# suous/RecNeXt

Hardware: AMD Instinct MI355X
Metric: images/sec RecNeXt-M3 224x224 bf16 (higher is better)
Workload: dtype bf16

## Files before the change

### recnext_amd/csrc/rcx_api.hip

```cpp
#include "../../include/recnext_amd.h"
#include "rcx_opts.h"
#include "rcx_launch.h"

#include <cstdarg>
#include <initializer_list>
#include <cstdio>
#include <cstdlib>

namespace {

thread_local char g_err[512] = "";

int fail(int code, const char* fmt, ...)
{
    va_list ap;
    va_start(ap, fmt);
    vsnprintf(g_err, sizeof(g_err), fmt, ap);
    va_end(ap);
    return code;
}

int hip_fail(hipError_t e, const char* what, const char* prefix = "")
{
    snprintf(g_err, sizeof(g_err), "%s%s: %s", prefix, what, hipGetErrorString(e));
// ... 935 lines not shown
    return e == hipSuccess ? 0 : hip_fail(e, "rcx_recattn_qkcore_fwd");
}

int rcx_recattn_down_qkcore_supported(int B, int H, int W, int C, int heads, int x_dtype)
{
    if (B <= 0 || H <= 0 || W <= 0 || C <= 0 || heads <= 0 || C % heads) return 0;
    return rcx::recattn_down_qkcore_applicable(B, H, W, C, heads, x_dtype) ? 1 : 0;
}

int rcx_recattn_down_qkcore_fwd(const void* x, const float* w_down_kkc, const float* b_down, const void* wqk_bf16, const float* bqk,
                                const float* w_pe_kkc, const float* b_pe, float* out, int B, int H, int W, int C, int heads, int x_dtype, void* stream)
{
    if (!x || !w_down_kkc || !wqk_bf16 || !bqk || !w_pe_kkc || !out) return fail(RCX_ERR_BAD_ARG, "rcx_recattn_down_qkcore_fwd: null pointer");
    if (B <= 0 || H <= 0 || W <= 0 || C <= 0 || heads <= 0) return fail(RCX_ERR_BAD_ARG, "non-positive extent B=%d H=%d W=%d C=%d heads=%d", B, H, W, C, heads);
    if (C % heads) return fail(RCX_ERR_BAD_ARG, "C=%d is not a multiple of heads=%d", C, heads);
    if (!known_dtype(x_dtype)) return fail(RCX_ERR_BAD_ARG, "unknown dtype %d", x_dtype);
    if (((size_t)wqk_bf16 & 15) || ((size_t)out & 15) || ((size_t)bqk & 15) || ((size_t)w_pe_kkc & 15) || ((size_t)b_pe & 15))
        return fail(RCX_ERR_BAD_ARG, "rcx_recattn_down_qkcore_fwd: wqk, bqk, w_pe_kkc, b_pe and out must be 16-byte aligned");
    if (!rcx::recattn_down_qkcore_applicable(B, H, W, C, heads, x_dtype))
        return fail(RCX_ERR_UNSUPPORTED, "rcx_recattn_down_qkcore_fwd: %d x %d plane, %d heads of %d, dtype %d: the one-launch form takes the 14 x 14 plane (1 .. 8 heads) "
                                         "and the 7 x 7 plane (1 .. 16 heads) of bf16 / f16 activations, heads of 4 .. 32 channels, or 2, 4 or 8 heads of 36 .. 64 in fours "
                                         "whose image fits the LDS (use rcx_dwconv2d_fwd + rcx_recattn_qkcore_fwd)",
                    H, W, heads, C / heads, x_dtype);
    hipError_t e = rcx::recattn_down_qkcore(x, w_down_kkc, b_down, wqk_bf16, bqk, w_pe_kkc, b_pe, out, B, H, C, heads, x_dtype, (hipStream_t)stream);
    return e == hipSuccess ? 0 : hip_fail(e, "rcx_recattn_down_qkcore_fwd");
}

int rcx_recattn2d_fwd_supported(int B, int H, int W, int C, int heads, int mode, int dtype)
{
    if (B <= 0 || H <= 0 || W <= 0 || C <= 0 || heads <= 0 || C % heads) return 0;
    return rcx::recattn2d_unit_applicable(B, H, W, C, heads, dtype, mode == RCX_MODE_NEAREST ? 1 : 0) ? 1 : 0;
}

int rcx_recattn2d_fwd(const void* x, void* y, const float* w_down_kkc, const float* b_down, const void* wqk_bf16, const float* bqk,
                      const float* w_pe_kkc, const float* b_pe, const float* w_conv_kkc, const float* b_conv,
                      int B, int H, int W, int C, int heads, int mode, int dtype, void* stream)
{
    if (!x || !y || !w_down_kkc || !wqk_bf16 || !bqk || !w_pe_kkc || !w_conv_kkc) return fail(RCX_ERR_BAD_ARG, "rcx_recattn2d_fwd: null pointer");
    if (B <= 0 || H <= 0 || W <= 0 || C <= 0 || heads <= 0) return fail(RCX_ERR_BAD_ARG, "non-positive extent B=%d H=%d W=%d C=%d heads=%d", B, H, W, C, heads);
    if (C % heads) return fail(RCX_ERR_BAD_ARG, "C=%d is not a multiple of heads=%d", C, heads);
    if (!known_dtype(dtype)) return fail(RCX_ERR_BAD_ARG, "unknown dtype %d", dtype);
    if (mode != RCX_MODE_BILINEAR && mode != RCX_MODE_NEAREST) return fail(RCX_ERR_BAD_ARG, "unknown mode %d", mode);
    if (((size_t)wqk_bf16 & 15) || ((size_t)bqk & 15) || ((size_t)w_pe_kkc & 15) || ((size_t)b_pe & 15))
        return fail(RCX_ERR_BAD_ARG, "rcx_recattn2d_fwd: wqk, bqk, w_pe_kkc and b_pe must be 16-byte aligned");
    if (!rcx::recattn2d_unit_applicable(B, H, W, C, heads, dtype, mode == RCX_MODE_NEAREST ? 1 : 0))
        return fail(RCX_ERR_UNSUPPORTED, "rcx_recattn2d_fwd: %d x %d plane, %d heads of %d, mode %d, dtype %d: the one-launch unit takes the 14 x 14 (1 .. 8 heads) and 7 x 7 (1 .. 16 heads) planes of bf16 / f16 "
                                         "activations, heads of 32 or 4 .. 28 channels (not above 32), nearest resize (use rcx_recattn_down_qkcore_fwd / rcx_dwconv2d_fwd + rcx_recattn_qkcore_fwd, then "
                                         "rcx_upadd_dwconv_fwd)", H, W, heads, C / heads, mode, dtype);
    hipError_t e = rcx::recattn2d_unit(x, w_down_kkc, b_down, wqk_bf16, bqk, w_pe_kkc, b_pe, w_conv_kkc, b_conv, y, B, H, C, heads, dtype, (hipStream_t)stream);
    return e == hipSuccess ? 0 : hip_fail(e, "rcx_recattn2d_fwd");
}

int rcx_stem_supported(int N, int H, int W, int CM, int CO, int dtype) { return rcx::stem_applicable(N, H, W, CM, CO, dtype) ? 1 : 0; }

size_t rcx_stem_pack_bytes(int CM, int CO) { return rcx::stem_pack_bytes(CM, CO); }

int rcx_stem_fwd(const void* x, void* y, const void* w1frag, const float* b1, const void* w2frag, const float* b2, int N, int H, int W, int CM, int CO, int dtype, void* stream)
{
    if (!x || !y || !w1frag || !b1 || !w2frag || !b2) return fail(RCX_ERR_BAD_ARG, "rcx_stem_fwd: null pointer");
    if (N <= 0 || H <= 0 || W <= 0 || CM <= 0 || CO <= 0) return fail(RCX_ERR_BAD_ARG, "non-positive extent N=%d H=%d W=%d CM=%d CO=%d", N, H, W, CM, CO);
    if (!known_dtype(dtype)) return fail(RCX_ERR_BAD_ARG, "unknown dtype %d", dtype);
    if (((size_t)x & 1) || ((size_t)y & 7) || ((size_t)w1frag & 15) || ((size_t)b1 & 15) || ((size_t)w2frag & 15) || ((size_t)b2 & 15))
        return fail(RCX_ERR_BAD_ARG, "rcx_stem_fwd: w1frag, b1, w2frag and b2 must be 16-byte aligned, y 8-byte aligned");
    if (!rcx::stem_applicable(N, H, W, CM, CO, dtype))
        return fail(RCX_ERR_UNSUPPORTED, "rcx_stem_fwd: no kernel for CM=%d CO=%d dtype %d (bf16; CM in {20, 24, 28, 32, 40}, CO %% 4 == 0, CO <= 96; one image of x below 2^31 bytes)", CM, CO, dtype);
    hipError_t e = rcx::stem_fwd(x, y, w1frag, b1, w2frag, b2, N, H, W, CM, CO, dtype, (hipStream_t)stream);
    return e == hipSuccess ? 0 : hip_fail(e, "rcx_stem_fwd");
}

int rcx_channel_mlp_supported(int M, int C, int H, int dtype) { return rcx::channel_mlp_applicable(M, C, H, dtype) ? 1 : 0; }

size_t rcx_channel_mlp_pack_bytes(int C, int H) { return rcx::channel_mlp_pack_bytes(C, H); }

int rcx_channel_mlp_fwd(const void* z, const void* x, void* y, const void* wfrag, const float* bias, int M, int C, int H, int dtype, void* stream)
{
    if (!z || !x || !y || !wfrag || !bias) return fail(RCX_ERR_BAD_ARG, "rcx_channel_mlp_fwd: null pointer");
    if (M <= 0 || C <= 0 || H <= 0) return fail(RCX_ERR_BAD_ARG, "non-positive extent M=%d C=%d H=%d", M, C, H);
    if (!known_dtype(dtype)) return fail(RCX_ERR_BAD_ARG, "unknown dtype %d", dtype);
    if (((size_t)z & 15) || ((size_t)x & 7) || ((size_t)y & 7) || ((size_t)wfrag & 15) || ((size_t)bias & 15))
        return fail(RCX_ERR_BAD_ARG, "rcx_channel_mlp_fwd: z, wfrag and bias must be 16-byte aligned, x and y 8-byte aligned");
    if (y == z || y == x) return fail(RCX_ERR_BAD_ARG, "rcx_channel_mlp_fwd: y must not alias its inputs");
    if (!rcx::channel_mlp_applicable(M, C, H, dtype))
        return fail(RCX_ERR_UNSUPPORTED, "rcx_channel_mlp_fwd: no kernel for M=%d C=%d H=%d dtype %d (bf16; (C, H) = (40 | 48, 96), (56 | 64, 128), (80, 160), (96, 192), (128, 256), (160, 320), "
                                         "(192, 384), (256, 512), (320, 640); M C 2 < 2^31)", M, C, H, dtype);
    hipError_t e = rcx::channel_mlp(z, x, y, wfrag, bias, M, C, H, dtype, (hipStream_t)stream);
    return e == hipSuccess ? 0 : hip_fail(e, "rcx_channel_mlp_fwd");
}

int rcx_ls_recattn_supported(int B, int H, int W, int C, int split, int heads, int dtype)
{
    return rcx::ls_recattn_applicable(B, H, W, C, split, heads, dtype) ? 1 : 0;
}

int rcx_ls_la3_supported(int B, int H, int W, int C, int split, int heads, int dtype)
{
    return rcx::ls_la3_applicable(B, H, W, C, split, heads, dtype) ? 1 : 0;
}

namespace {
bool any_misaligned(std::initializer_list<const void*> ps)
{
    for (const void* p : ps)
        if ((size_t)p & 15) return true;
    return false;
}
}

int rcx_ls_recattn_fwd(const void* x, void* r, void* t, const float* w_rep, const float* b_rep, const float* w_down_kkc, const float* b_down,
                       const float* wqT, const float* bq, const float* wkT, const float* bk, const float* w_pe_kkc, const float* b_pe,
                       const float* w_conv_kkc, const float* b_conv, int B, int H, int W, int C, int split, int heads, int dtype, void* stream)
{
    if (!x || !r || !t || !w_rep || !b_rep || !w_down_kkc || !b_down || !wqT || !bq || !wkT || !bk || !w_pe_kkc || !b_pe || !w_conv_kkc || !b_conv)
        return fail(RCX_ERR_BAD_ARG, "rcx_ls_recattn_fwd: null pointer");
    if (B <= 0 || H <= 0 || W <= 0 || C <= 0 || split <= 0 || heads <= 0)
        return fail(RCX_ERR_BAD_ARG, "non-positive extent B=%d H=%d W=%d C=%d split=%d heads=%d", B, H, W, C, split, heads);
    if (!known_dtype(dtype)) return fail(RCX_ERR_BAD_ARG, "unknown dtype %d", dtype);
    if (r == x || t == x || r == t) return fail(RCX_ERR_BAD_ARG, "rcx_ls_recattn_fwd: r and t must alias neither x nor each other");
    if (any_misaligned({x, r, t, w_rep, b_rep, w_down_kkc, b_down, wqT, bq, wkT, bk, w_pe_kkc, b_pe, w_conv_kkc, b_conv}))
        return fail(RCX_ERR_BAD_ARG, "rcx_ls_recattn_fwd: every tensor must be 16-byte aligned");
    if (!rcx::ls_recattn_applicable(B, H, W, C, split, heads, dtype))
        return fail(RCX_ERR_UNSUPPORTED, "rcx_ls_recattn_fwd: %d x %d plane, C=%d, split=%d, %d heads: one head, C and split multiples of 4, and an image whose slice "
                                         "mixer fits the LDS", H, W, C, split, heads);
    hipError_t e = rcx::ls_recattn_fwd(x, r, t, w_rep, b_rep, w_down_kkc, b_down, wqT, bq, wkT, bk, w_pe_kkc, b_pe, w_conv_kkc, b_conv,
                                       B, H, W, C, split, dtype, (hipStream_t)stream);
    return e == hipSuccess ? 0 : hip_fail(e, "rcx_ls_recattn_fwd");
}

int rcx_ls_la3_fwd(const void* x, void* r, void* t, const float* w_rep, const float* b_rep, const float* wqT, const float* bq,
                   const float* wkT, const float* bk, const float* w_pe_kkc, const float* b_pe, int B, int H, int W, int C, int split, int heads,
                   int dtype, void* stream)
{
    if (!x || !r || !t || !w_rep || !b_rep || !wqT || !bq || !wkT || !bk || !w_pe_kkc || !b_pe) return fail(RCX_ERR_BAD_ARG, "rcx_ls_la3_fwd: null pointer");
    if (B <= 0 || H <= 0 || W <= 0 || C <= 0 || split <= 0 || heads <= 0)
        return fail(RCX_ERR_BAD_ARG, "non-positive extent B=%d H=%d W=%d C=%d split=%d heads=%d", B, H, W, C, split, heads);
    if (!known_dtype(dtype)) return fail(RCX_ERR_BAD_ARG, "unknown dtype %d", dtype);
    if (r == x || t == x || r == t) return fail(RCX_ERR_BAD_ARG, "rcx_ls_la3_fwd: r and t must alias neither x nor each other");
    if (any_misaligned({x, r, t, w_rep, b_rep, wqT, bq, wkT, bk, w_pe_kkc, b_pe}))
        return fail(RCX_ERR_BAD_ARG, "rcx_ls_la3_fwd: every tensor must be 16-byte aligned");
    if (!rcx::ls_la3_applicable(B, H, W, C, split, heads, dtype))
        return fail(RCX_ERR_UNSUPPORTED, "rcx_ls_la3_fwd: %d x %d plane, C=%d, split=%d, %d heads: at most 64 tokens, C and split multiples of 4, split a multiple "
                                         "of 2 heads", H, W, C, split, heads);
    hipError_t e = rcx::ls_la3_fwd(x, r, t, w_rep, b_rep, wqT, bq, wkT, bk, w_pe_kkc, b_pe, B, H, W, C, split, heads, dtype, (hipStream_t)stream);
    return e == hipSuccess ? 0 : hip_fail(e, "rcx_ls_la3_fwd");
}

int rcx_ls_recattn_tiled_supported(int B, int H, int W, int C, int split, int heads, int dtype)
{
    return rcx::ls_recattn_tiled_applicable(B, H, W, C, split, heads, dtype) ? 1 : 0;
}

int rcx_ls_la3_tiled_supported(int B, int H, int W, int C, int split, int heads, int dtype)
{
    return rcx::ls_la3_tiled_applicable(B, H, W, C, split, heads, dtype) ? 1 : 0;
}

size_t rcx_ls_recattn_tiled_workspace_bytes(int B, int H, int W, int C, int split, int heads, int dtype)
{
    return rcx::ls_recattn_tiled_workspace_bytes(B, H, W, C, split, heads, dtype);
}

size_t rcx_ls_la3_tiled_workspace_bytes(int B, int H, int W, int C, int split, int heads, int dtype)
{
    return rcx::ls_la3_tiled_workspace_bytes(B, H, W, C, split, heads, dtype);
}

namespace {
int check_ls_tiled(const char* fn, std::initializer_list<const void*> ps, const void* x, const void* r, const void* t, const void* workspace,
// ... 98 lines not shown
```

### recnext_amd/csrc/rcx_mlp.hip

```cpp
#include "rcx_common.h"
#include "rcx_launch.h"
#include "rcx_gelu.h"

namespace rcx {
namespace mlp {

typedef float f32x16 __attribute__((ext_vector_type(16)));
typedef float f32x4q __attribute__((ext_vector_type(4)));
typedef float f32x2q __attribute__((ext_vector_type(2)));
typedef __bf16 bf16x8 __attribute__((ext_vector_type(8)));
typedef __bf16 bf16x4 __attribute__((ext_vector_type(4)));
typedef unsigned u32x4q __attribute__((ext_vector_type(4)));
typedef unsigned u32x2q __attribute__((ext_vector_type(2)));

__device__ __forceinline__ void wave_sync()
{
    __builtin_amdgcn_fence(__ATOMIC_RELEASE, "wavefront");
    __builtin_amdgcn_wave_barrier();
    __builtin_amdgcn_fence(__ATOMIC_ACQUIRE, "wavefront");
}

template <int KS1, int CT, int RD>
__device__ __forceinline__ void hidden_tile_ring(const u32x4q* Lc, const float* b1t, int lane, int h, const bf16x8 (&zb)[KS1], f32x16 (&d2)[CT])
{
    constexpr int R1 = KS1 < RD ? KS1 : RD, N2 = 2 * CT, R2 = N2 < RD ? N2 : RD;
    u32x4q ring[RD];
#pragma unroll
    for (int j = 0; j < R1; ++j) ring[j] = Lc[j * 64 + lane];
    f32x16 d1;
#pragma unroll
    for (int i = 0; i < 16; ++i) d1[i] = 0.f;
#pragma unroll
    for (int ks = 0; ks < KS1; ++ks) {
        const bf16x8 a = __builtin_bit_cast(bf16x8, ring[ks % R1]);
        if (ks + R1 < KS1) ring[ks % R1] = Lc[(ks + R1) * 64 + lane];
        d1 = __builtin_amdgcn_mfma_f32_32x32x16_bf16(a, zb[ks], d1, 0, 0, 0);
    }
#pragma unroll
    for (int f = 0; f < R2; ++f) ring[f] = Lc[(KS1 + 2 * (f % CT) + f / CT) * 64 + lane];
    bf16x8 hb[2];
    gelu_f32x2 gv[8];
#pragma unroll
    for (int g = 0; g < 4; ++g) {
        const f32x4q bb = *reinterpret_cast<const f32x4q*>(b1t + 8 * g + 4 * h);
        gv[2 * g] = gelu_f32x2{d1[4 * g] + bb.x, d1[4 * g + 1] + bb.y};
        gv[2 * g + 1] = gelu_f32x2{d1[4 * g + 2] + bb.z, d1[4 * g + 3] + bb.w};
    }
    {
        gelu_f32x2 ga[4] = {gv[0], gv[1], gv[2], gv[3]}, gb[4] = {gv[4], gv[5], gv[6], gv[7]};
        gelu2x_batch<4>(ga);
        gelu2x_batch<4>(gb);
#pragma unroll
        for (int i = 0; i < 4; ++i) { gv[i] = ga[i]; gv[4 + i] = gb[i]; }
    }
#pragma unroll
    for (int g = 0; g < 4; ++g) {
        hb[g >> 1][4 * (g & 1) + 0] = (__bf16)gv[2 * g].x; hb[g >> 1][4 * (g & 1) + 1] = (__bf16)gv[2 * g].y;
        hb[g >> 1][4 * (g & 1) + 2] = (__bf16)gv[2 * g + 1].x; hb[g >> 1][4 * (g & 1) + 3] = (__bf16)gv[2 * g + 1].y;
    }
#pragma unroll
    for (int f = 0; f < N2; ++f) {
        const bf16x8 a = __builtin_bit_cast(bf16x8, ring[f % R2]);
        if (f + R2 < N2) ring[f % R2] = Lc[(KS1 + 2 * ((f + R2) % CT) + (f + R2) / CT) * 64 + lane];
        d2[f % CT] = __builtin_amdgcn_mfma_f32_32x32x16_bf16(a, hb[f / CT], d2[f % CT], 0, 0, 0);
    }
}


template <int KS1, int HT, int CT, int NW, int WPS, bool KX, bool OX, bool STAGED>
__global__ void __launch_bounds__(64 * NW, WPS)
k_channel_mlp(const bf16_t* __restrict__ z, const bf16_t* __restrict__ xres, bf16_t* __restrict__ y, const u32x4q* __restrict__ wfrag, const float* __restrict__ bias,
              int M, int C, int ntiles)
{
    extern __shared__ __attribute__((aligned(16))) unsigned char lds_raw[];
    constexpr int NF = HT * KS1 + CT * 2 * HT;
    const u32x4q* const Lf = reinterpret_cast<const u32x4q*>(lds_raw);
    const float* const Lb1 = reinterpret_cast<const float*>(lds_raw + (size_t)NF * 1024);
    const float* const Lb2 = Lb1 + 32 * HT;
    {
        u32x4q* Lw = reinterpret_cast<u32x4q*>(lds_raw);
        for (int i = threadIdx.x; i < NF * 64; i += 64 * NW) Lw[i] = wfrag[i];
        float* Lb = reinterpret_cast<float*>(lds_raw + (size_t)NF * 1024);
        for (int i = threadIdx.x; i < 32 * (HT + CT); i += 64 * NW) Lb[i] = bias[i];
    }
    __syncthreads();
// ... 269 lines not shown
        const u32x4q* src = wfrag + (size_t)chunk * NCH * 64 + threadIdx.x;
        u32x4q* dst = Lring + (size_t)slot * NCH * 64 + wv * 64;
#pragma unroll
        for (int i = 0; i < PER; ++i)
            __builtin_amdgcn_global_load_lds((__attribute__((address_space(1))) void*)(src + i * NT), (__attribute__((address_space(3))) void*)(dst + i * NT), 16, 0, 0);
    };
    constexpr int VM_ALL = 0x70, VM_NEXT = 0x70 | (PER & 15) | ((PER >> 4) << 14);
    fill(0, 0);
    fill(1, 1);
    for (int i = threadIdx.x; i < 32 * (HT + CT); i += NT) Lb1[i] = bias[i];
    const unsigned nbytes = (unsigned)M * (unsigned)C * 2u;
    const __amdgpu_buffer_rsrc_t zsrc = __builtin_amdgcn_make_buffer_rsrc((void*)z, 0, nbytes, 0x00020000);
    const __amdgpu_buffer_rsrc_t xsrc = __builtin_amdgcn_make_buffer_rsrc((void*)xres, 0, nbytes, 0x00020000);
    const __amdgpu_buffer_rsrc_t ysrc = __builtin_amdgcn_make_buffer_rsrc((void*)y, 0, nbytes, 0x00020000);
    const unsigned zo0 = (unsigned)(lane >> 3) * RB + 16u * (lane & 7), za0 = (unsigned)(lane >> 3) * ZP + 16u * (lane & 7);
    const unsigned ot = lane >> 2, ob = 16u * (lane & 3);
    if (!(__builtin_popcount(wv) & 1)) __builtin_amdgcn_s_setprio(1);
    int slot = 0;
    for (int block = blockIdx.x; block < nblocks; block += gridDim.x) {
        const unsigned base = (unsigned)(32 * (block * NW + wave)) * (unsigned)RB;
        const bool more = block + (int)gridDim.x < nblocks;
        bf16x8 zb[KS1];
        {
            u32x4q zq[KS1];
#pragma unroll
            for (int i = 0; i < KS1; ++i)
                zq[i] = __builtin_bit_cast(u32x4q, __builtin_amdgcn_raw_buffer_load_b128(zsrc, (int)(base + zo0 + 8u * RB * (i % KH) + RBH * (i / KH)), 0, 0));
#pragma unroll
            for (int q = 0; q < ZH; ++q) {
#pragma unroll
                for (int i = 0; i < KH; ++i) *reinterpret_cast<u32x4q*>(Lt + za0 + 8 * ZP * i) = zq[q * KH + i];
                wave_sync();
#pragma unroll
                for (int k = 0; k < KH; ++k) zb[q * KH + k] = __builtin_bit_cast(bf16x8, *reinterpret_cast<const u32x4q*>(Lt + r * ZP + 32 * k + 16 * h));
                wave_sync();
            }
        }
        f32x16 d2[CT];
#pragma unroll
        for (int ct = 0; ct < CT; ++ct)
#pragma unroll
            for (int i = 0; i < 16; ++i) d2[ct][i] = 0.f;
#pragma unroll 1
        for (int ht = 0; ht < HT; ++ht) {
            if (ht + 1 < HT || more) __builtin_amdgcn_s_waitcnt(VM_NEXT);
            else __builtin_amdgcn_s_waitcnt(VM_ALL);
            __builtin_amdgcn_s_barrier();
            if (ht + 2 < HT || more) fill((ht + 2) % HT, slot == 0 ? 2 : slot - 1);
            hidden_tile_ring<KS1, CT, 4>(Lring + (size_t)slot * NCH * 64, Lb1 + 32 * ht, lane, h, zb, d2);
            slot = slot == NS - 1 ? 0 : slot + 1;
        }
        u32x4q xq[CT][2];
#pragma unroll
        for (int ct = 0; ct < CT; ++ct)
#pragma unroll
            for (int j = 0; j < 2; ++j)
                xq[ct][j] = __builtin_bit_cast(u32x4q, __builtin_amdgcn_raw_buffer_load_b128(xsrc, (int)(base + (16u * j + ot) * RB + 64u * ct + ob), 0, 0));
#pragma unroll
        for (int ct = 0; ct < CT; ++ct) {
#pragma unroll
            for (int g = 0; g < 4; ++g) {
                const f32x4q bb = *reinterpret_cast<const f32x4q*>(Lb2 + 32 * ct + 8 * g + 4 * h);
                *reinterpret_cast<f32x4q*>(Lt + r * OP + 4 * (8 * g + 4 * h)) =
                    f32x4q{d2[ct][4 * g] + bb.x, d2[ct][4 * g + 1] + bb.y, d2[ct][4 * g + 2] + bb.z, d2[ct][4 * g + 3] + bb.w};
            }
            wave_sync();
#pragma unroll
            for (int j = 0; j < 2; ++j) {
                const unsigned char* src = Lt + (16 * j + ot) * OP + 2 * ob;
                const f32x4q lo = *reinterpret_cast<const f32x4q*>(src), hi = *reinterpret_cast<const f32x4q*>(src + 16);
                const u32x4q xv = xq[ct][j];
                bf16x8 o;
                o[0] = (__bf16)(lo.x + __uint_as_float(xv.x << 16)); o[1] = (__bf16)(lo.y + __uint_as_float(xv.x & 0xffff0000u));
                o[2] = (__bf16)(lo.z + __uint_as_float(xv.y << 16)); o[3] = (__bf16)(lo.w + __uint_as_float(xv.y & 0xffff0000u));
                o[4] = (__bf16)(hi.x + __uint_as_float(xv.z << 16)); o[5] = (__bf16)(hi.y + __uint_as_float(xv.z & 0xffff0000u));
                o[6] = (__bf16)(hi.z + __uint_as_float(xv.w << 16)); o[7] = (__bf16)(hi.w + __uint_as_float(xv.w & 0xffff0000u));
                __builtin_amdgcn_raw_buffer_store_b128(__builtin_bit_cast(u32x4q, o), ysrc, (int)(base + (16u * j + ot) * RB + 64u * ct + ob), 0, 0);
            }
            wave_sync();
        }
    }
}

}

static bool mlp_shape(int C, int H, int* ks1, int* ht, int* ct)
{
    if (C <= 0 || H <= 0 || C % 8 || H % 32) return false;
    *ks1 = (C + 15) / 16; *ht = H / 32; *ct = (C + 31) / 32;
    if (C > 128 && (*ct & 1)) ++*ct;
    return true;
}

bool channel_mlp_applicable(int M, int C, int H, int dtype)
{
    int ks1, ht, ct;
    if (dtype != 1 || M <= 0 || !mlp_shape(C, H, &ks1, &ht, &ct)) return false;
    if ((unsigned long long)M * C * 2 >= (1ull << 31)) return false;
    if (C == 256 && ht == 16) return true;
    if (C == 192 && ht == 12) return true;
    if ((C == 160 && ht == 10) || (C == 320 && ht == 20)) return true;
    return (ks1 == 4 && ht == 4 && ct == 2) || (C == 128 && ht == 8) || (ks1 == 3 && ht == 3 && ct == 2) || (C == 96 && ht == 6) || (C == 80 && ht == 5);
}

size_t channel_mlp_pack_bytes(int C, int H)
{
    int ks1, ht, ct;
    if (!mlp_shape(C, H, &ks1, &ht, &ct)) return 0;
    return (size_t)(ht * ks1 + ct * 2 * ht) * 1024;
}

template <int KS1, int HT, int CT, bool KX, bool OX>
static hipError_t launch_mlp(const void* z, const void* x, void* y, const void* wfrag, const float* bias, int M, int C, int ncu, hipStream_t s)
{
    constexpr size_t lds = (size_t)(HT * KS1 + CT * 2 * HT) * 1024 + sizeof(float) * 32 * (HT + CT);
    static_assert(lds <= 160 * 1024, "the weights must fit the LDS");
    constexpr int NW = CT <= 2 ? 12 : 8, WPS = NW / 4;
    constexpr bool STAGED = CT <= 2;
    constexpr size_t stage = STAGED ? (size_t)NW * 32 * ((32 * KS1 + 16) > (128 * CT + 16) ? (32 * KS1 + 16) : (128 * CT + 16)) : 0;
    if ((C == 16 * KS1) != KX || (C == 32 * CT) != OX) return hipErrorInvalidConfiguration;
    auto kfn = mlp::k_channel_mlp<KS1, HT, CT, NW, WPS, KX, OX, STAGED>;
    static_assert(lds + stage <= 160 * 1024, "weights + the waves' images must fit the LDS");
    RCX_SET_LDS_ONCE(kfn, lds + stage);
    const int ntiles = (M + 31) / 32;
    int grid = ncu;
    if (grid * NW > ntiles) grid = (ntiles + NW - 1) / NW;
    hipLaunchKernelGGL(kfn, dim3((unsigned)grid), dim3(64 * NW), lds + stage, s, (const bf16_t*)z, (const bf16_t*)x, (bf16_t*)y, (const mlp::u32x4q*)wfrag, bias, M, C, ntiles);
    return hipGetLastError();
}

template <int KS1, int HT, int CT, int NW, int ZH = 1, bool ZPF = true>
static hipError_t launch_mlp_stream(const void* z, const void* x, void* y, const void* wfrag, const float* bias, int M, int C, int ncu, hipStream_t s)
{
    constexpr int NCH = KS1 + 2 * CT, ZP = 32 * KS1 / ZH + 16, OP = 256 + 16, IMG = 32 * (ZP > OP ? ZP : OP);
    constexpr size_t lds = (size_t)2 * NCH * 1024 + sizeof(float) * 32 * (HT + CT) + (size_t)NW * IMG;
    static_assert(lds <= 160 * 1024, "the ring and the waves' images must fit the LDS");
    static_assert(CT % 2 == 0 && 32 * CT >= 16 * KS1 && 32 * (CT - 2) < 16 * KS1, "output tiles: the channel count rounded up to a multiple of 64");
    if (C != 16 * KS1) return hipErrorInvalidConfiguration;
    auto kfn = mlp::k_channel_mlp_stream<KS1, HT, CT, NW, NW / 4, ZH, ZPF>;
    RCX_SET_LDS_ONCE(kfn, lds);
    const int nblocks = (M + 32 * NW - 1) / (32 * NW);
    const int grid = nblocks < ncu ? nblocks : ncu;
    hipLaunchKernelGGL(kfn, dim3((unsigned)grid), dim3(64 * NW), lds, s, (const bf16_t*)z, (const bf16_t*)x, (bf16_t*)y, (const mlp::u32x4q*)wfrag, bias, M, C, nblocks);
    return hipGetLastError();
}

static hipError_t launch_mlp_pair256(const void* z, const void* x, void* y, const void* wfrag, const float* bias, int M, int C, int ncu, hipStream_t s)
{
    constexpr int KS1 = 16, HT = 16, CT = 8, NCH = KS1 + 2 * CT, IMG = 32 * (128 + 16);
    constexpr size_t lds = (size_t)3 * NCH * 1024 + sizeof(float) * 32 * (HT + CT) + (size_t)8 * IMG;
    static_assert(lds <= 160 * 1024, "the ring and the waves' images must fit the LDS");
    if (C != 16 * KS1) return hipErrorInvalidConfiguration;
    auto kfn = mlp::k_channel_mlp_pair<KS1, HT, CT>;
    RCX_SET_LDS_ONCE(kfn, lds);
    const int nblocks = (M + 255) / 256;
    const int grid = nblocks < ncu ? nblocks : ncu;
    hipLaunchKernelGGL(kfn, dim3((unsigned)grid), dim3(512), lds, s, (const bf16_t*)z, (const bf16_t*)x, (bf16_t*)y, (const mlp::u32x4q*)wfrag, bias, M, C, nblocks);
    return hipGetLastError();
}

hipError_t channel_mlp(const void* z, const void* x, void* y, const void* wfrag, const float* bias, int M, int C, int H, int dtype, hipStream_t s)
{
    int ks1, ht, ct;
    if (!channel_mlp_applicable(M, C, H, dtype) || !mlp_shape(C, H, &ks1, &ht, &ct)) return hipErrorInvalidConfiguration;
    static std::atomic<int> cus[RCX_MAX_DEVICES];
    int dev = 0, ncu = 256;
    if (hipGetDevice(&dev) == hipSuccess && dev >= 0 && dev < RCX_MAX_DEVICES) {
        ncu = cus[dev].load(std::memory_order_relaxed);
        if (ncu <= 0) {
            int v = 0;
            ncu = hipDeviceGetAttribute(&v, hipDeviceAttributeMultiprocessorCount, dev) == hipSuccess && v > 0 ? v : 256;
            cus[dev].store(ncu, std::memory_order_relaxed);
        }
    }
    if (C == 256 && ht == 16) return launch_mlp_pair256(z, x, y, wfrag, bias, M, C, ncu, s);
    if (C == 192 && ht == 12) return launch_mlp_stream<12, 12, 6, 4>(z, x, y, wfrag, bias, M, C, ncu, s);
    if (C == 160 && ht == 10) return launch_mlp_stream<10, 10, 6, 4>(z, x, y, wfrag, bias, M, C, ncu, s);
    if (C == 320 && ht == 20) return launch_mlp_stream<20, 20, 10, 4, 2, false>(z, x, y, wfrag, bias, M, C, ncu, s);
    if (ks1 == 4 && ht == 4) return C == 64 ? launch_mlp<4, 4, 2, true, true>(z, x, y, wfrag, bias, M, C, ncu, s)
                                            : launch_mlp<4, 4, 2, false, false>(z, x, y, wfrag, bias, M, C, ncu, s);
    if (ks1 == 8 && ht == 8) {
        if (C != 128) return hipErrorInvalidConfiguration;
        return launch_mlp_stream<8, 8, 4, 8>(z, x, y, wfrag, bias, M, C, ncu, s);
    }
    if (ks1 == 3 && ht == 3) return C == 48 ? launch_mlp<3, 3, 2, true, false>(z, x, y, wfrag, bias, M, C, ncu, s)
                                            : launch_mlp<3, 3, 2, false, false>(z, x, y, wfrag, bias, M, C, ncu, s);
    if (ks1 == 6 && ht == 6) return C == 96 ? launch_mlp<6, 6, 3, true, true>(z, x, y, wfrag, bias, M, C, ncu, s) : hipErrorInvalidConfiguration;
    if (ks1 == 5 && ht == 5) return C == 80 ? launch_mlp<5, 5, 3, true, false>(z, x, y, wfrag, bias, M, C, ncu, s) : hipErrorInvalidConfiguration;
    return hipErrorInvalidConfiguration;
}

}
```

Baseline: 109,800.

## Add fused channel-MLP kernel for C=512 with streamed weight fragments

After: 113,200 (median of 6 runs). 3.1% higher.

```diff
diff --git a/recnext_amd/csrc/rcx_api.hip b/recnext_amd/csrc/rcx_api.hip
--- a/recnext_amd/csrc/rcx_api.hip
+++ b/recnext_amd/csrc/rcx_api.hip
@@ -1041,7 +1041,7 @@
     if (y == z || y == x) return fail(RCX_ERR_BAD_ARG, "rcx_channel_mlp_fwd: y must not alias its inputs");
     if (!rcx::channel_mlp_applicable(M, C, H, dtype))
         return fail(RCX_ERR_UNSUPPORTED, "rcx_channel_mlp_fwd: no kernel for M=%d C=%d H=%d dtype %d (bf16; (C, H) = (40 | 48, 96), (56 | 64, 128), (80, 160), (96, 192), (128, 256), (160, 320), "
-                                         "(192, 384), (256, 512), (320, 640); M C 2 < 2^31)", M, C, H, dtype);
+                                         "(192, 384), (256, 512), (320, 640), (512, 1024) from a minimum M upward; M C 2 < 2^31)", M, C, H, dtype);
     hipError_t e = rcx::channel_mlp(z, x, y, wfrag, bias, M, C, H, dtype, (hipStream_t)stream);
     return e == hipSuccess ? 0 : hip_fail(e, "rcx_channel_mlp_fwd");
 }
diff --git a/recnext_amd/csrc/rcx_mlp.hip b/recnext_amd/csrc/rcx_mlp.hip
--- a/recnext_amd/csrc/rcx_mlp.hip
+++ b/recnext_amd/csrc/rcx_mlp.hip
@@ -1,6 +1,7 @@
 #include "rcx_common.h"
 #include "rcx_launch.h"
 #include "rcx_gelu.h"
+#include <type_traits>
 
 namespace rcx {
 namespace mlp {
@@ -436,6 +437,178 @@
     }
 }
 
+
+template <int KS1, int HT, int CT, int RD>
+__global__ void __launch_bounds__(512, 2)
+k_channel_mlp_wide(const bf16_t* __restrict__ z, const bf16_t* __restrict__ xres, bf16_t* __restrict__ y, const u32x4q* __restrict__ wfrag, const float* __restrict__ bias, int M)
+{
+    extern __shared__ __attribute__((aligned(16))) unsigned char lds_raw[];
+    constexpr int NW = 8, NT = 64 * NW, SH = 8, NST = HT / SH, NCH = KS1 + 2 * CT, NF = KS1 + 4 * SH;
+    static_assert(CT == 2 * NW && HT % SH == 0 && SH == NW && NF % RD == 0 && KS1 % RD == 0 && KS1 % 8 == 0, "a hidden tile (phase A) and two output tiles (phase B) per wave");
+    constexpr int RB = 32 * KS1, OP = 256 + 16, IMG = 32 * OP;
+    constexpr int ZBYTES = 2 * KS1 * 1024, XBYTES = SH * 4 * 1024;
+    static_assert(NW * IMG <= ZBYTES + XBYTES, "the output images alias the z fragments and exchange buffer 0");
+    u32x4q* const Lz = reinterpret_cast<u32x4q*>(lds_raw);
+    u32x4q* const Lx = reinterpret_cast<u32x4q*>(lds_raw + ZBYTES);
+    float* const Lb1 = reinterpret_cast<float*>(lds_raw + ZBYTES + 2 * XBYTES);
+    const float* const Lb2 = Lb1 + 32 * HT;
+    const int lane = threadIdx.x & 63, r = lane & 31, h = lane >> 5;
+    const int wv = __builtin_amdgcn_readfirstlane(threadIdx.x >> 6);
+    auto frag = [&](int s, int i) -> u32x4q {
+        const int ht = SH * s + (i < KS1 ? wv : (i - KS1) >> 2);
+        const int f = i < KS1 ? i : KS1 + 4 * wv + 2 * ((i - KS1) & 1) + (((i - KS1) >> 1) & 1);
+        return wfrag[((size_t)ht * NCH + f) * 64 + lane];
+    };
+    u32x4q ring[RD];
+#pragma unroll
+    for (int i = 0; i < RD; ++i) ring[i] = frag(0, i);
+    const unsigned nbytes = (unsigned)M * (unsigned)RB;
+    const __amdgpu_buffer_rsrc_t zsrc = __builtin_amdgcn_make_buffer_rsrc((void*)z, 0, nbytes, 0x00020000);
+    const __amdgpu_buffer_rsrc_t xsrc = __builtin_amdgcn_make_buffer_rsrc((void*)xres, 0, nbytes, 0x00020000);
+    const __amdgpu_buffer_rsrc_t ysrc = __builtin_amdgcn_make_buffer_rsrc((void*)y, 0, nbytes, 0x00020000);
+    const unsigned base = blockIdx.x * 64u * RB;
+    {
+        const unsigned go = base + (8u * wv + (lane & 7)) * RB + 16u * (lane >> 3);
+        u32x4q zq[KS1 / 4];
+#pragma unroll
+        for (int j = 0; j < KS1 / 4; ++j) zq[j] = __builtin_bit_cast(u32x4q, __builtin_amdgcn_raw_buffer_load_b128(zsrc, (int)(go + 128u * j), 0, 0));
+        for (int i = threadIdx.x; i < 32 * (HT + CT); i += NT) Lb1[i] = bias[i];
+        u32x4q* const dst = Lz + ((wv >> 2) * KS1 + (lane >> 4)) * 64 + ((lane >> 3) & 1) * 32 + 8 * (wv & 3) + (lane & 7);
+#pragma unroll
+        for (int j = 0; j < KS1 / 4; ++j) dst[4 * j * 64] = zq[j];
+    }
+    __syncthreads();
+    if (!(__builtin_popcount(wv) & 1)) __builtin_amdgcn_s_setprio(1);
+    constexpr int LGKM0 = 0xC07F;
+    f32x16 d2[2][2];
+#pragma unroll
+    for (int c2 = 0; c2 < 2; ++c2)
+#pragma unroll
+        for (int tt = 0; tt < 2; ++tt)
+#pragma unroll
+            for (int i = 0; i < 16; ++i) d2[c2][tt][i] = 0.f;
+    const unsigned ot = lane >> 3, ob = 16u * (lane & 7);
+    u32x4q xq[2][4];
+    auto step = [&](int s, auto last_c) {
+        constexpr bool LAST = decltype(last_c)::value;
+        const int sn = LAST ? 0 : s + 1;
+        f32x16 d1[2];
+#pragma unroll
+        for (int tt = 0; tt < 2; ++tt)
+#pragma unroll
+            for (int i = 0; i < 16; ++i) d1[tt][i] = 0.f;
+        constexpr int BD = 2;
+        u32x4q zb[BD][2];
+#pragma unroll
+        for (int k = 0; k < BD; ++k)
+#pragma unroll
+            for (int tt = 0; tt < 2; ++tt) zb[k][tt] = Lz[(tt * KS1 + k) * 64 + lane];
+#pragma unroll
+        for (int ks = 0; ks < KS1; ++ks) {
+            const bf16x8 a = __builtin_bit_cast(bf16x8, ring[ks % RD]);
+            ring[ks % RD] = frag(s, ks + RD);
+            const bf16x8 b0 = __builtin_bit_cast(bf16x8, zb[ks % BD][0]), b1 = __builtin_bit_cast(bf16x8, zb[ks % BD][1]);
+            if (ks + BD < KS1) {
+#pragma unroll
+                for (int tt = 0; tt < 2; ++tt) zb[ks % BD][tt] = Lz[(tt * KS1 + ks + BD) * 64 + lane];
+            }
+            d1[0] = __builtin_amdgcn_mfma_f32_32x32x16_bf16(a, b0, d1[0], 0, 0, 0);
+            d1[1] = __builtin_amdgcn_mfma_f32_32x32x16_bf16(a, b1, d1[1], 0, 0, 0);
+            __builtin_amdgcn_sched_barrier(0);
+        }
+        const float* const b1t = Lb1 + 32 * (SH * s + wv);
+        u32x4q* const Lw = Lx + (size_t)(s & 1) * (XBYTES / 16) + wv * 4 * 64 + lane;
+#pragma unroll
+        for (int tt = 0; tt < 2; ++tt) {
+            gelu_f32x2 gv[8];
+#pragma unroll
+            for (int g = 0; g < 4; ++g) {
+                const f32x4q bb = *reinterpret_cast<const f32x4q*>(b1t + 8 * g + 4 * h);
+                gv[2 * g] = gelu_f32x2{d1[tt][4 * g] + bb.x, d1[tt][4 * g + 1] + bb.y};
+                gv[2 * g + 1] = gelu_f32x2{d1[tt][4 * g + 2] + bb.z, d1[tt][4 * g + 3] + bb.w};
+            }
+            {
+                gelu_f32x2 ga[4] = {gv[0], gv[1], gv[2], gv[3]}, gb[4] = {gv[4], gv[5], gv[6], gv[7]};
+                gelu2x_batch<4>(ga);
+                gelu2x_batch<4>(gb);
+#pragma unroll
+                for (int i = 0; i < 4; ++i) { gv[i] = ga[i]; gv[4 + i] = gb[i]; }
+            }
+            bf16x8 hb[2];
+#pragma unroll
+            for (int g = 0; g < 4; ++g) {
+                hb[g >> 1][4 * (g & 1) + 0] = (__bf16)gv[2 * g].x; hb[g >> 1][4 * (g & 1) + 1] = (__bf16)gv[2 * g].y;
+                hb[g >> 1][4 * (g & 1) + 2] = (__bf16)gv[2 * g + 1].x; hb[g >> 1][4 * (g & 1) + 3] = (__bf16)gv[2 * g + 1].y;
+            }
+            Lw[(2 * tt) * 64] = __builtin_bit_cast(u32x4q, hb[0]);
+            Lw[(2 * tt + 1) * 64] = __builtin_bit_cast(u32x4q, hb[1]);
+        }
+        __builtin_amdgcn_s_waitcnt(LGKM0);
+        __builtin_amdgcn_s_barrier();
+        if constexpr (LAST) {
+#pragma unroll
+            for (int tt = 0; tt < 2; ++tt)
+#pragma unroll
+                for (int j = 0; j < 4; ++j)
+                    xq[tt][j] = __builtin_bit_cast(u32x4q, __builtin_amdgcn_raw_buffer_load_b128(xsrc, (int)(base + (32u * tt + 8u * j + ot) * RB + 128u * wv + ob), 0, 0));
+        }
+        const u32x4q* const Lr = Lx + (size_t)(s & 1) * (XBYTES / 16) + lane;
+        u32x4q hq[2][2][2];
+#pragma unroll
+        for (int tt = 0; tt < 2; ++tt)
+#pragma unroll
+            for (int q = 0; q < 2; ++q) hq[0][tt][q] = Lr[(2 * tt + q) * 64];
+#pragma unroll
+        for (int hl = 0; hl < SH; ++hl) {
+            if (hl + 1 < SH) {
+#pragma unroll
+                for (int tt = 0; tt < 2; ++tt)
+#pragma unroll
+                    for (int q = 0; q < 2; ++q) hq[(hl + 1) & 1][tt][q] = Lr[((hl + 1) * 4 + 2 * tt + q) * 64];
+            }
+#pragma unroll
+            for (int j = 0; j < 4; ++j) {
+                const int i = KS1 + 4 * hl + j, c2 = j & 1, q = j >> 1;
+                const bf16x8 a = __builtin_bit_cast(bf16x8, ring[i % RD]);
+                if (i + RD < NF) ring[i % RD] = frag(s, i + RD);
+                else if (!LAST) ring[i % RD] = frag(sn, i + RD - NF);
+                d2[c2][0] = __builtin_amdgcn_mfma_f32_32x32x16_bf16(a, __builtin_bit_cast(bf16x8, hq[hl & 1][0][q]), d2[c2][0], 0, 0, 0);
+                d2[c2][1] = __builtin_amdgcn_mfma_f32_32x32x16_bf16(a, __builtin_bit_cast(bf16x8, hq[hl & 1][1][q]), d2[c2][1], 0, 0, 0);
+                __builtin_amdgcn_sched_barrier(0);
+            }
+        }
+    };
+#pragma unroll 1
+    for (int s = 0; s < NST - 1; ++s) step(s, std::false_type{});
+    step(NST - 1, std::true_type{});
+    unsigned char* const Lt = lds_raw + (size_t)wv * IMG;
+#pragma unroll
+    for (int tt = 0; tt < 2; ++tt) {
+#pragma unroll
+        for (int c2 = 0; c2 < 2; ++c2)
+#pragma unroll
+            for (int g = 0; g < 4; ++g) {
+                const f32x4q bb = *reinterpret_cast<const f32x4q*>(Lb2 + 32 * (2 * wv + c2) + 8 * g + 4 * h);
+                *reinterpret_cast<f32x4q*>(Lt + r * OP + 4 * (32 * c2 + 8 * g + 4 * h)) =
+                    f32x4q{d2[c2][tt][4 * g] + bb.x, d2[c2][tt][4 * g + 1] + bb.y, d2[c2][tt][4 * g + 2] + bb.z, d2[c2][tt][4 * g + 3] + bb.w};
+            }
+        wave_sync();
+#pragma unroll
+        for (int j = 0; j < 4; ++j) {
+            const unsigned char* src = Lt + (8 * j + ot) * OP + 2 * ob;
+            const f32x4q lo = *reinterpret_cast<const f32x4q*>(src), hi = *reinterpret_cast<const f32x4q*>(src + 16);
+            const u32x4q xv = xq[tt][j];
+            bf16x8 o;
+            o[0] = (__bf16)(lo.x + __uint_as_float(xv.x << 16)); o[1] = (__bf16)(lo.y + __uint_as_float(xv.x & 0xffff0000u));
+            o[2] = (__bf16)(lo.z + __uint_as_float(xv.y << 16)); o[3] = (__bf16)(lo.w + __uint_as_float(xv.y & 0xffff0000u));
+            o[4] = (__bf16)(hi.x + __uint_as_float(xv.z << 16)); o[5] = (__bf16)(hi.y + __uint_as_float(xv.z & 0xffff0000u));
+            o[6] = (__bf16)(hi.z + __uint_as_float(xv.w << 16)); o[7] = (__bf16)(hi.w + __uint_as_float(xv.w & 0xffff0000u));
+            __builtin_amdgcn_raw_buffer_store_b128(__builtin_bit_cast(u32x4q, o), ysrc, (int)(base + (32u * tt + 8u * j + ot) * RB + 128u * wv + ob), 0, 0);
+        }
+        wave_sync();
+    }
+}
+
 }
 
 static bool mlp_shape(int C, int H, int* ks1, int* ht, int* ct)
@@ -446,11 +619,14 @@
     return true;
 }
 
+static constexpr int MLP512_MIN_TOKENS = 2048;
+
 bool channel_mlp_applicable(int M, int C, int H, int dtype)
 {
     int ks1, ht, ct;
     if (dtype != 1 || M <= 0 || !mlp_shape(C, H, &ks1, &ht, &ct)) return false;
     if ((unsigned long long)M * C * 2 >= (1ull << 31)) return false;
+    if (C == 512 && ht == 32) return M >= MLP512_MIN_TOKENS;
     if (C == 256 && ht == 16) return true;
     if (C == 192 && ht == 12) return true;
     if ((C == 160 && ht == 10) || (C == 320 && ht == 20)) return true;
@@ -513,6 +689,18 @@
     return hipGetLastError();
 }
 
+static hipError_t launch_mlp_wide512(const void* z, const void* x, void* y, const void* wfrag, const float* bias, int M, int C, hipStream_t s)
+{
+    constexpr int KS1 = 32, HT = 32, CT = 16;
+    constexpr size_t lds = (size_t)2 * KS1 * 1024 + (size_t)2 * 8 * 4 * 1024 + sizeof(float) * 32 * (HT + CT);
+    static_assert(lds <= 160 * 1024, "the z fragments, the exchange buffers and the biases must fit the LDS");
+    if (C != 16 * KS1) return hipErrorInvalidConfiguration;
+    auto kfn = mlp::k_channel_mlp_wide<KS1, HT, CT, 8>;
+    RCX_SET_LDS_ONCE(kfn, lds);
+    hipLaunchKernelGGL(kfn, dim3((unsigned)((M + 63) / 64)), dim3(512), lds, s, (const bf16_t*)z, (const bf16_t*)x, (bf16_t*)y, (const mlp::u32x4q*)wfrag, bias, M);
+    return hipGetLastError();
+}
+
 hipError_t channel_mlp(const void* z, const void* x, void* y, const void* wfrag, const float* bias, int M, int C, int H, int dtype, hipStream_t s)
 {
     int ks1, ht, ct;
@@ -527,6 +715,7 @@
             cus[dev].store(ncu, std::memory_order_relaxed);
         }
     }
+    if (C == 512 && ht == 32) return launch_mlp_wide512(z, x, y, wfrag, bias, M, C, s);
     if (C == 256 && ht == 16) return launch_mlp_pair256(z, x, y, wfrag, bias, M, C, ncu, s);
     if (C == 192 && ht == 12) return launch_mlp_stream<12, 12, 6, 4>(z, x, y, wfrag, bias, M, C, ncu, s);
     if (C == 160 && ht == 10) return launch_mlp_stream<10, 10, 6, 4>(z, x, y, wfrag, bias, M, C, ncu, s);
```
